# chrischoy/DeepGlobalRegistration

Measured on NVIDIA B200. Metric: scan_pairs_per_sec, higher is better.
Workload: dtype f32

## Files before the change

### deepglobalregistration_b200/csrc/knn_tc.cu

```cuda
#include <stdlib.h>

#include "common.cuh"
#include "tc_common.cuh"

namespace {

using namespace tc;

constexpr int kLoadWarps = 4;
constexpr int kLoadThreads = kLoadWarps * 32;
constexpr int kMmaWarpK = kLoadWarps;
constexpr int kEpiWarps = 8;
constexpr int kThreadsK = (kLoadWarps + 1 + kEpiWarps) * 32;
constexpr int kRowsA = 128;
constexpr int kColsB = 256;
constexpr int kATile = kRowsA * 128;
constexpr int kBTile = kColsB * 128;
constexpr int kCandCap = 16;
constexpr int kEpiThreads = kEpiWarps * 32;
constexpr size_t kCandBytes = (size_t)2 * kCandCap * kEpiThreads * 4;
constexpr int kPass1Stride = 1;

__global__ void row_norms_kernel(const float* __restrict__ f, int64_t n, int c, float* __restrict__ n2,
                                 unsigned* __restrict__ max_bits) {
  int64_t row = ((int64_t)blockIdx.x * blockDim.x + threadIdx.x) >> 3;
  int sub = threadIdx.x & 7;
  float s = 0.f;
  if (row < n)
    for (int k = sub; k < c; k += 8) {
      float v = f[row * c + k];
      s = fmaf(v, v, s);
    }
  s += __shfl_xor_sync(0xffffffffu, s, 1);
  s += __shfl_xor_sync(0xffffffffu, s, 2);
  s += __shfl_xor_sync(0xffffffffu, s, 4);
  if (row < n && sub == 0) {
    n2[row] = s;
    if (max_bits != nullptr) atomicMax(max_bits, __float_as_uint(s));
  }
}

__global__ void knn_tc_init_kernel(unsigned* __restrict__ rowmin_bits, unsigned long long* __restrict__ packed,
                                   int64_t n0, unsigned* max_bits) {
  int64_t i = (int64_t)blockIdx.x * blockDim.x + threadIdx.x;
  if (i < n0) {
    rowmin_bits[i] = 0x7f800000u;
    packed[i] = ~0ull;
  }
  if (i == 0) *max_bits = 0u;
}

__device__ __forceinline__ float knn_error_bound(float na, float nb, bool fine) {
  const float rel = fine ? 4e-6f : (0.0009765625f * 1.25f + 4e-5f);
  return rel * na * nb + 1e-6f * (na + nb) * (na + nb) + 1e-7f;
}
__global__ void knn_tc_threshold_kernel(const unsigned* __restrict__ rowmin_bits, const float* __restrict__ na2,
                                        const unsigned* __restrict__ nb2_max_bits, int64_t n0, int fine,
                                        float* __restrict__ thr) {
  int64_t i = (int64_t)blockIdx.x * blockDim.x + threadIdx.x;
  if (i >= n0) return;
  const float na = sqrtf(na2[i]), nb = sqrtf(__uint_as_float(*nb2_max_bits));
  const float e = knn_error_bound(na, nb, fine != 0);
  thr[i] = 0.5f * (__uint_as_float(rowmin_bits[i]) + 4.f * e - na2[i]);
}

struct KnnShared {
  unsigned long long full[2];
  unsigned long long acc_full[2];
  unsigned long long acc_empty[2];
  uint32_t tmem_base;
  float nb[2][kColsB];
};

__device__ __forceinline__ void round_store(float4 v, unsigned char* tile, int row, int piece) {
  float4 h;
  h.x = tf32_round(v.x); h.y = tf32_round(v.y); h.z = tf32_round(v.z); h.w = tf32_round(v.w);
  *reinterpret_cast<float4*>(tile + row * 128 + ((piece ^ (row & 7)) << 4)) = h;
}

__device__ __forceinline__ void split_store2(float4 v, unsigned char* hi_tile, unsigned char* lo_tile, int row, int piece) {
  float4 h, l;
  h.x = tf32_round(v.x); h.y = tf32_round(v.y); h.z = tf32_round(v.z); h.w = tf32_round(v.w);
  l.x = v.x - h.x; l.y = v.y - h.y; l.z = v.z - h.z; l.w = v.w - h.w;
  const int off = row * 128 + ((piece ^ (row & 7)) << 4);
  *reinterpret_cast<float4*>(hi_tile + off) = h;
  *reinterpret_cast<float4*>(lo_tile + off) = l;
}

template <int C>
__device__ __noinline__ void knn_exact_candidate(const float* __restrict__ f0, const float* __restrict__ f1,
                                                 int gi, int j, float& best_s, float& best_d2, int& best_j) {
  const float4* a = reinterpret_cast<const float4*>(f0 + (size_t)gi * C);
  const float4* b = reinterpret_cast<const float4*>(f1 + (size_t)j * C);
  float d2 = 0.f;
#pragma unroll
  for (int k = 0; k < C / 4; ++k) {
    const float4 x = __ldg(a + k), y = __ldg(b + k);
    float df = x.x - y.x; d2 = fmaf(df, df, d2);
    df = x.y - y.y; d2 = fmaf(df, df, d2);
    df = x.z - y.z; d2 = fmaf(df, df, d2);
    df = x.w - y.w; d2 = fmaf(df, df, d2);
  }
  if (d2 < best_d2) {
    const float sq = sqrtf(d2 + 1e-7f);
    if (sq < best_s) {
      best_s = sq;
      best_d2 = d2;
      best_j = j;
    }
  }
}

template <int C>
__device__ __noinline__ void knn_exact_candidate_unordered(const float* __restrict__ f0, const float* __restrict__ f1,
                                                           int gi, int j, float& best_s, float& best_d2, int& best_j) {
  const float4* a = reinterpret_cast<const float4*>(f0 + (size_t)gi * C);
  const float4* b = reinterpret_cast<const float4*>(f1 + (size_t)j * C);
  float d2 = 0.f;
#pragma unroll
  for (int k = 0; k < C / 4; ++k) {
    const float4 x = __ldg(a + k), y = __ldg(b + k);
    float df = x.x - y.x; d2 = fmaf(df, df, d2);
    df = x.y - y.y; d2 = fmaf(df, df, d2);
    df = x.z - y.z; d2 = fmaf(df, df, d2);
    df = x.w - y.w; d2 = fmaf(df, df, d2);
  }
  const float sq = sqrtf(d2 + 1e-7f);
  if (sq < best_s || (sq == best_s && j < best_j)) {
    best_s = sq;
    best_j = j;
  }
  best_d2 = fminf(best_d2, d2);
}

__device__ __forceinline__ void tc_ld32_issue(uint32_t taddr, uint32_t (&v)[32]) {
  asm volatile(
      "tcgen05.ld.sync.aligned.32x32b.x32.b32 "
      "{%0, %1, %2, %3, %4, %5, %6, %7, %8, %9, %10, %11, %12, %13, %14, %15, "
      "%16, %17, %18, %19, %20, %21, %22, %23, %24, %25, %26, %27, %28, %29, %30, %31}, [%32];"
      : "=r"(v[0]), "=r"(v[1]), "=r"(v[2]), "=r"(v[3]), "=r"(v[4]), "=r"(v[5]), "=r"(v[6]), "=r"(v[7]),
        "=r"(v[8]), "=r"(v[9]), "=r"(v[10]), "=r"(v[11]), "=r"(v[12]), "=r"(v[13]), "=r"(v[14]),
        "=r"(v[15]), "=r"(v[16]), "=r"(v[17]), "=r"(v[18]), "=r"(v[19]), "=r"(v[20]), "=r"(v[21]),
        "=r"(v[22]), "=r"(v[23]), "=r"(v[24]), "=r"(v[25]), "=r"(v[26]), "=r"(v[27]), "=r"(v[28]),
        "=r"(v[29]), "=r"(v[30]), "=r"(v[31])
      : "r"(taddr)
// ... 194 lines not shown
        atomicMin(packed + gi, ((unsigned long long)__float_as_uint(best_s) << 32) | (unsigned)best_j);
    }
  } else {
    const int lane_grp = warp & 3;
    const int half = (warp - kLoadWarps - 1) >> 2;
    const int r = lane_grp * 32 + lane;
    const int gi = row0 + r;
    const bool valid = gi < n0;
    float th = (PASS == 2 && valid) ? thr[gi] : -__int_as_float(0x7f800000);
    const float na2_i = (PASS == 2 && valid) ? na2[gi] : 0.f;
    const float e4 = (PASS == 2 && valid)
                         ? 4.f * knn_error_bound(sqrtf(na2_i), sqrtf(__uint_as_float(*nb2_max_bits)), kFine)
                         : 0.f;
    float rmin = __int_as_float(0x7f800000);
    float best_s = __int_as_float(0x7f800000), best_d2 = best_s;
    int best_j = 0x7fffffff;
    for (int it = 0; it < n_tiles; ++it) {
      const int s = it & 1;
      const uint32_t ph = (it >> 1) & 1;
      const int j0 = col_begin + it * kTS * kColsB + half * 128;
      mbar_wait(smem_u32(&sh.acc_full[s]), ph);
      tc_fence_after();
      const uint32_t taddr = tmem_base + (uint32_t)s * kColsB + half * 128 + ((uint32_t)(lane_grp * 32) << 16);
      const float* hb = sh.nb[s] + half * 128;
      uint32_t va[32], vb[32];
      tc_ld32_issue(taddr, va);
#pragma unroll
      for (int cc = 0; cc < 4; ++cc) {
        tc_ld_wait();
        uint32_t(&cur)[32] = (cc & 1) ? vb : va;
        uint32_t(&nxt)[32] = (cc & 1) ? va : vb;
        if (cc < 3) tc_ld32_issue(taddr + (cc + 1) * 32, nxt);
        const int jc = j0 + cc * 32;
        if (jc < col_end) {
          if (jc + 32 <= col_end) {
            float cmin = __int_as_float(0x7f800000);
#pragma unroll
            for (int q = 0; q < 32; ++q) cmin = fminf(cmin, hb[cc * 32 + q] - __uint_as_float(cur[q]));
            if (PASS == 1) {
              rmin = fminf(rmin, cmin);
            } else if (cmin <= th) {
#pragma unroll
              for (int q = 0; q < 32; ++q) {
                const float g = hb[cc * 32 + q] - __uint_as_float(cur[q]);
                if (g <= th) {
                  knn_exact_candidate<C>(f0, f1, gi, jc + q, best_s, best_d2, best_j);
                  th = fminf(th, 0.5f * (best_d2 + e4 - na2_i));
                }
              }
            }
          } else {
#pragma unroll
            for (int q = 0; q < 32; ++q) {
              const float g = hb[cc * 32 + q] - __uint_as_float(cur[q]);
              if (jc + q < col_end) {
                if (PASS == 1) rmin = fminf(rmin, g);
                else if (g <= th) {
                  knn_exact_candidate<C>(f0, f1, gi, jc + q, best_s, best_d2, best_j);
                  th = fminf(th, 0.5f * (best_d2 + e4 - na2_i));
                }
              }
            }
          }
        }
      }
      tc_fence_before();
      mbar_arrive(smem_u32(&sh.acc_empty[s]));
    }
    if (valid) {
      if (PASS == 1) {
        atomicMin(rowmin_bits + gi, __float_as_uint(fmaxf(fmaf(2.f, rmin, na2[gi]), 0.f)));
      } else if (best_j != 0x7fffffff) {
        atomicMin(packed + gi, ((unsigned long long)__float_as_uint(best_s) << 32) | (unsigned)best_j);
      }
    }
  }
  tc_fence_before();
  __syncthreads();
  if (warp == kMmaWarpK) {
    asm volatile("tcgen05.dealloc.cta_group::1.sync.aligned.b32 %0, %1;" ::"r"(tmem_base), "r"(512u) : "memory");
  }
}

__global__ void knn_tc_unpack_kernel(const unsigned long long* __restrict__ packed, int64_t n,
                                     int32_t* __restrict__ idx, float* __restrict__ dist) {
  int64_t i = (int64_t)blockIdx.x * blockDim.x + threadIdx.x;
  if (i >= n) return;
  unsigned long long p = packed[i];
  idx[i] = (int32_t)(p & 0xffffffffu);
  if (dist != nullptr) dist[i] = __uint_as_float((unsigned)(p >> 32));
}

template <int C>
int32_t launch_knn_tc_single(const float* f0, int64_t n0, const float* f1, int64_t n1, float* na2, float* nb2,
                             unsigned* max_bits, unsigned long long* packed, cudaStream_t st) {
  constexpr int kChunks = C / 32;
  const size_t smem = sizeof(KnnShared) + 1024 + (size_t)kChunks * kATile + 2 * (size_t)kChunks * kBTile + kCandBytes;
  DGR_ENSURE_SMEM((knn_tc_kernel<C, 3, false>), smem);
  const int row_tiles = (int)((n0 + kRowsA - 1) / kRowsA);
  const int col_tiles = (int)((n1 + kColsB - 1) / kColsB);
  int splits = (148 * 4 + row_tiles - 1) / row_tiles;
  if (splits > col_tiles) splits = col_tiles;
  if (splits < 1) splits = 1;
  const int cols_per_split = ((col_tiles + splits - 1) / splits) * kColsB;
  splits = (int)((n1 + cols_per_split - 1) / cols_per_split);
  dim3 grid(row_tiles, splits);
  knn_tc_kernel<C, 3, false><<<grid, kThreadsK, smem, st>>>(f0, (int)n0, f1, (int)n1, na2, nb2, cols_per_split,
                                                            nullptr, nullptr, packed, max_bits);
  return DGR_OK;
}

template <int C, bool kFine>
int32_t launch_knn_tc(const float* f0, int64_t n0, const float* f1, int64_t n1, float* na2, float* nb2,
                      unsigned* rowmin, float* thr, unsigned* max_bits, unsigned long long* packed,
                      cudaStream_t st) {
  constexpr int kChunks = C / 32;
  constexpr int kParts = kFine ? 2 : 1;
  const size_t smem = sizeof(KnnShared) + 1024 + (size_t)kParts * kChunks * kATile + 2 * (size_t)kParts * kChunks * kBTile;
  DGR_ENSURE_SMEM((knn_tc_kernel<C, 1, kFine>), smem);
  DGR_ENSURE_SMEM((knn_tc_kernel<C, 2, kFine>), smem);
  const int row_tiles = (int)((n0 + kRowsA - 1) / kRowsA);
  const int col_tiles = (int)((n1 + kColsB - 1) / kColsB);
  int splits = (148 * 4 + row_tiles - 1) / row_tiles;
  if (splits > col_tiles) splits = col_tiles;
  if (splits < 1) splits = 1;
  const int cols_per_split = ((col_tiles + splits - 1) / splits) * kColsB;
  splits = (int)((n1 + cols_per_split - 1) / cols_per_split);
  dim3 grid(row_tiles, splits);
  knn_tc_kernel<C, 1, kFine><<<grid, kThreadsK, smem, st>>>(f0, (int)n0, f1, (int)n1, na2, nb2, cols_per_split,
                                                            rowmin, thr, packed, max_bits);
  knn_tc_threshold_kernel<<<dgr_blocks(n0, 256), 256, 0, st>>>(rowmin, na2, max_bits, n0, kFine ? 1 : 0, thr);
  knn_tc_kernel<C, 2, kFine><<<grid, kThreadsK, smem, st>>>(f0, (int)n0, f1, (int)n1, na2, nb2, cols_per_split,
                                                            rowmin, thr, packed, max_bits);
  return DGR_OK;
}

}

extern "C" {

int64_t dgr_knn_tc_ws_elems(int64_t n0, int64_t n1) { return 3 * n0 + n1 + 8; }

int32_t dgr_knn_tc_supported(int32_t c) { return (c == 32 || c == 64) ? 1 : 0; }

int32_t dgr_knn_top1_tc(const float* f0, int64_t n0, const float* f1, int64_t n1, int32_t c,
                        uint64_t* packed_ws, float* ws, int32_t* idx, float* dist, void* stream) {
  DGR_ARG_CHECK(dgr_knn_tc_supported(c), "channel count not supported by the tensor-core kNN");
  DGR_ARG_CHECK(n1 >= 1 || n0 == 0, "F1 must not be empty");
  DGR_ARG_CHECK(n0 < (1ll << 31) && n1 < (1ll << 31), "too many rows");
  if (n0 == 0) return DGR_OK;
  cudaStream_t st = (cudaStream_t)stream;
  float* na2 = ws;
  float* thr = ws + n0;
  unsigned* rowmin = reinterpret_cast<unsigned*>(ws + 2 * n0);
  float* nb2 = ws + 3 * n0;
  unsigned* max_bits = reinterpret_cast<unsigned*>(ws + 3 * n0 + n1);
  unsigned long long* packed = reinterpret_cast<unsigned long long*>(packed_ws);
  knn_tc_init_kernel<<<dgr_blocks(n0, 256), 256, 0, st>>>(rowmin, packed, n0, max_bits);
  row_norms_kernel<<<dgr_blocks(n0 * 8, 256), 256, 0, st>>>(f0, n0, c, na2, nullptr);
  row_norms_kernel<<<dgr_blocks(n1 * 8, 256), 256, 0, st>>>(f1, n1, c, nb2, max_bits);
  static const bool coarse = getenv("DGR_KNN_FINE") == nullptr;
  static const bool single = getenv("DGR_KNN_SWEEPS") != nullptr && atoi(getenv("DGR_KNN_SWEEPS")) == 1;
  if (single) {
    int32_t rc1 = (c == 32) ? launch_knn_tc_single<32>(f0, n0, f1, n1, na2, nb2, max_bits, packed, st)
                            : launch_knn_tc_single<64>(f0, n0, f1, n1, na2, nb2, max_bits, packed, st);
    if (rc1 != DGR_OK) return rc1;
    knn_tc_unpack_kernel<<<dgr_blocks(n0, 256), 256, 0, st>>>(packed, n0, idx, dist);
    dgr_note_launches(5);
    DGR_LAUNCH_CHECK();
    return DGR_OK;
  }
  int32_t rc = (c == 32) ? (coarse ? launch_knn_tc<32, false>(f0, n0, f1, n1, na2, nb2, rowmin, thr, max_bits, packed, st)
                                   : launch_knn_tc<32, true>(f0, n0, f1, n1, na2, nb2, rowmin, thr, max_bits, packed, st))
                         : launch_knn_tc<64, false>(f0, n0, f1, n1, na2, nb2, rowmin, thr, max_bits, packed, st);
  if (rc != DGR_OK) return rc;
  knn_tc_unpack_kernel<<<dgr_blocks(n0, 256), 256, 0, st>>>(packed, n0, idx, dist);
  dgr_note_launches(7);
  DGR_LAUNCH_CHECK();
  return DGR_OK;
}

}
```

### deepglobalregistration_b200/csrc/spconv_tc.cu

```cuda
#include <cuda_fp16.h>
#include <stdlib.h>

#include "common.cuh"
#include "tc_common.cuh"

namespace {

using namespace tc;

#ifdef DGR_GATHER_CG
#define DGR_GATHER_LOAD(p) __ldcg(p)
#else
#define DGR_GATHER_LOAD(p) __ldg(p)
#endif

#define DGR_TRY_RC(expr)             \
  do {                              \
    int32_t rc__ = (expr);          \
    if (rc__ != DGR_OK) return rc__; \
  } while (0)

constexpr int kLoaderWarps = 8;
constexpr int kLoaderThreads = kLoaderWarps * 32;
constexpr int kMmaWarp = kLoaderWarps;
constexpr int kThreadsTC = (kLoaderWarps + 5) * 32;
constexpr int kTileM = 128;
constexpr int kChunk = 32;
constexpr int kATileBytes = kTileM * 128;

__device__ __forceinline__ void split_store(float4 v, unsigned char* hi_tile, unsigned char* lo_tile,
                                            uint32_t off) {
  float4 h, l;
  h.x = tf32_round(v.x); h.y = tf32_round(v.y); h.z = tf32_round(v.z); h.w = tf32_round(v.w);
  l.x = v.x - h.x; l.y = v.y - h.y; l.z = v.z - h.z; l.w = v.w - h.w;
  *reinterpret_cast<float4*>(hi_tile + off) = h;
  *reinterpret_cast<float4*>(lo_tile + off) = l;
}

__device__ __forceinline__ void split_store_f16(float4 a, float4 b, float sx, unsigned char* hi_tile,
                                                unsigned char* lo_tile, uint32_t off) {
  const float x[8] = {a.x * sx, a.y * sx, a.z * sx, a.w * sx, b.x * sx, b.y * sx, b.z * sx, b.w * sx};
  uint32_t h[4], l[4];
#pragma unroll
  for (int i = 0; i < 4; ++i) {
    const __half2 hh = __floats2half2_rn(x[2 * i], x[2 * i + 1]);
    const float2 hf = __half22float2(hh);
    const __half2 ll = __floats2half2_rn(x[2 * i] - hf.x, x[2 * i + 1] - hf.y);
    h[i] = *reinterpret_cast<const uint32_t*>(&hh);
    l[i] = *reinterpret_cast<const uint32_t*>(&ll);
  }
  *reinterpret_cast<uint4*>(hi_tile + off) = make_uint4(h[0], h[1], h[2], h[3]);
  *reinterpret_cast<uint4*>(lo_tile + off) = make_uint4(l[0], l[1], l[2], l[3]);
}
__device__ __forceinline__ float f16_scale_for(float amax) {
  const uint32_t b = __float_as_uint(amax);
  const int e = (int)((b >> 23) & 255u);
  if (e == 0 || e == 255) return 1.f;
  int se = 14 - (e - 127) + 127;
  se = se < 1 ? 1 : (se > 254 ? 254 : se);
  return __uint_as_float((uint32_t)se << 23);
}

__device__ __forceinline__ uint32_t cluster_ctarank() {
  uint32_t r;
  asm volatile("mov.u32 %0, %%cluster_ctarank;" : "=r"(r));
  return r;
}
__device__ __forceinline__ void cluster_sync_all() {
  asm volatile("barrier.cluster.arrive.release.aligned;" ::: "memory");
  asm volatile("barrier.cluster.wait.acquire.aligned;" ::: "memory");
}
__device__ __forceinline__ void bulk_g2s_multicast(uint32_t dst_smem, const void* src, uint32_t bytes,
                                                   uint32_t bar, uint16_t mask) {
  asm volatile(
      "cp.async.bulk.shared::cluster.global.mbarrier::complete_tx::bytes.multicast::cluster [%0], [%1], %2, [%3], %4;"
      ::"r"(dst_smem), "l"(src), "r"(bytes), "r"(bar), "h"(mask)
      : "memory");
}
__device__ __forceinline__ void tc_commit_multicast(uint32_t bar, uint16_t mask) {
  asm volatile(
      "tcgen05.commit.cta_group::1.mbarrier::arrive::one.shared::cluster.multicast::cluster.b64 [%0], %1;" ::"r"(bar),
      "h"(mask)
      : "memory");
}
__device__ __forceinline__ void mbar_arrive_expect_tx(uint32_t bar, uint32_t bytes) {
  asm volatile("mbarrier.arrive.expect_tx.shared::cta.b64 _, [%0], %1;" ::"r"(bar), "r"(bytes) : "memory");
}
__device__ __forceinline__ void mbar_expect_tx(uint32_t bar, uint32_t bytes) {
  asm volatile("mbarrier.expect_tx.relaxed.cta.shared::cta.b64 [%0], %1;" ::"r"(bar), "r"(bytes) : "memory");
}
__device__ __forceinline__ void bulk_g2s(uint32_t dst_smem, const void* src, uint32_t bytes, uint32_t bar) {
  asm volatile("cp.async.bulk.shared::cluster.global.mbarrier::complete_tx::bytes [%0], [%1], %2, [%3];" ::"r"(
                   dst_smem),
               "l"(src), "r"(bytes), "r"(bar)
               : "memory");
}


__device__ __forceinline__ void scatter32_lines(unsigned char* stg, int lane, float* __restrict__ out, int cout,
                                                int col, int j, const uint32_t (&v)[32]) {
#pragma unroll
  for (int q = 0; q < 8; ++q)
    *reinterpret_cast<uint4*>(stg + lane * 128 + ((q ^ (lane & 7)) << 4)) =
        make_uint4(v[4 * q], v[4 * q + 1], v[4 * q + 2], v[4 * q + 3]);
  __syncwarp();
  const int p = lane & 7, rsub = lane >> 3;
#pragma unroll
  for (int k = 0; k < 8; ++k) {
    const int R = rsub + 4 * k;
    const int jr = __shfl_sync(0xffffffffu, j, R);
    const float4 x = *reinterpret_cast<const float4*>(stg + R * 128 + ((p ^ (R & 7)) << 4));
    if (jr >= 0) red_add_v4(out + (size_t)jr * cout + col + p * 4, x.x, x.y, x.z, x.w);
  }
  __syncwarp();
}
__device__ __forceinline__ void scatter32_rows(float* __restrict__ out, int cout, int col, int j,
                                               const uint32_t (&v)[32]) {
  if (j >= 0) {
    float* dst = out + (size_t)j * cout + col;
#pragma unroll
    for (int q = 0; q < 8; ++q)
      red_add_v4(dst + 4 * q, __uint_as_float(v[4 * q]), __uint_as_float(v[4 * q + 1]),
                 __uint_as_float(v[4 * q + 2]), __uint_as_float(v[4 * q + 3]));
  }
}
constexpr int kEpiStageBytes = 4 * 4096;

struct TcShared {
  unsigned long long full[4];
  unsigned long long full_lo[4];
  unsigned long long empty[4];
  unsigned long long acc_full[2];
  unsigned long long acc_empty[2];
  uint32_t tmem_base;
};

template <int kCluster, int kPD>
__global__ void __launch_bounds__(kThreadsTC, 1)
spconv_tc_kernel(const float* __restrict__ in_feat, int cin, const float* __restrict__ wt, int cout,
                 const int32_t* __restrict__ in_idx, const int32_t* __restrict__ out_idx,
                 const int32_t* __restrict__ kofs, const int32_t* __restrict__ tile_k,
                 const int32_t* __restrict__ tile_start, int n_tiles, int n_stages, int tmem_cols,
                 int passes, int epi, float* __restrict__ out) {
  extern __shared__ __align__(16) unsigned char smem_dyn[];
  TcShared& sh = *reinterpret_cast<TcShared*>(smem_dyn);
  unsigned char* stage0 = reinterpret_cast<unsigned char*>(
      (reinterpret_cast<uintptr_t>(smem_dyn) + sizeof(TcShared) + 1023) & ~(uintptr_t)1023);
  const int b_tile_bytes = cout * 128;
  const int stage_bytes = 2 * kATileBytes + 2 * b_tile_bytes;
  const int t = threadIdx.x;
  const int warp = t >> 5, lane = t & 31;
  const int n_chunks = cin / kChunk;
  const uint32_t acc_stride = (uint32_t)tmem_cols >> 1;

  if (t == 0) {
    for (int s = 0; s < n_stages; ++s) {
      mbar_init(smem_u32(&sh.full[s]), kLoaderThreads);
      mbar_init(smem_u32(&sh.full_lo[s]), 1);
      mbar_init(smem_u32(&sh.empty[s]), kCluster);
    }
    for (int b = 0; b < 2; ++b) {
      mbar_init(smem_u32(&sh.acc_full[b]), 1);
      mbar_init(smem_u32(&sh.acc_empty[b]), 128);
    }
    asm volatile("fence.mbarrier_init.release.cluster;" ::: "memory");
  }
  if (warp == kMmaWarp) {
    asm volatile("tcgen05.alloc.cta_group::1.sync.aligned.shared::cta.b32 [%0], %1;" ::"r"(
                     smem_u32(&sh.tmem_base)),
                 "r"((uint32_t)tmem_cols)
                 : "memory");
    asm volatile("tcgen05.relinquish_alloc_permit.cta_group::1.sync.aligned;" ::: "memory");
  }
  tc_fence_before();
  __syncthreads();
  if (kCluster > 1) cluster_sync_all();
  tc_fence_after();
  const uint32_t tmem_base = sh.tmem_base;
// ... 920 lines not shown
```

### deepglobalregistration_b200/csrc/tc_common.cuh

```cuda
#pragma once
#include <cuda_runtime.h>
#include <stdint.h>

namespace tc {

__device__ __forceinline__ uint32_t smem_u32(const void* p) {
  return (uint32_t)__cvta_generic_to_shared(p);
}
__device__ __forceinline__ void mbar_init(uint32_t bar, uint32_t count) {
  asm volatile("mbarrier.init.shared::cta.b64 [%0], %1;" ::"r"(bar), "r"(count) : "memory");
}
__device__ __forceinline__ void mbar_arrive(uint32_t bar) {
  asm volatile("mbarrier.arrive.shared::cta.b64 _, [%0];" ::"r"(bar) : "memory");
}
__device__ __forceinline__ bool mbar_try_wait(uint32_t bar, uint32_t parity) {
  uint32_t ok;
  asm volatile(
      "{\n\t.reg .pred p;\n\t"
      "mbarrier.try_wait.parity.shared::cta.b64 p, [%1], %2;\n\t"
      "selp.u32 %0, 1, 0, p;\n\t}"
      : "=r"(ok)
      : "r"(bar), "r"(parity)
      : "memory");
  return ok != 0;
}
__device__ __forceinline__ void mbar_wait(uint32_t bar, uint32_t parity) {
  while (!mbar_try_wait(bar, parity)) {
  }
}
__device__ __forceinline__ void fence_proxy_async() {
  asm volatile("fence.proxy.async.shared::cta;" ::: "memory");
}
__device__ __forceinline__ void tc_fence_before() {
  asm volatile("tcgen05.fence::before_thread_sync;" ::: "memory");
}
__device__ __forceinline__ void tc_fence_after() {
  asm volatile("tcgen05.fence::after_thread_sync;" ::: "memory");
}
__device__ __forceinline__ void tc_commit(uint32_t bar) {
  asm volatile("tcgen05.commit.cta_group::1.mbarrier::arrive::one.shared::cluster.b64 [%0];" ::"r"(bar)
               : "memory");
}
__device__ __forceinline__ void tc_mma_tf32(uint32_t tmem_d, uint64_t adesc, uint64_t bdesc, uint32_t idesc,
                                            uint32_t accumulate) {
  asm volatile(
      "{\n\t.reg .pred p;\n\t"
      "setp.ne.b32 p, %4, 0;\n\t"
      "tcgen05.mma.cta_group::1.kind::tf32 [%0], %1, %2, %3, p;\n\t}"
      ::"r"(tmem_d), "l"(adesc), "l"(bdesc), "r"(idesc), "r"(accumulate)
      : "memory");
}
__device__ __forceinline__ void tc_mma_tf32_ts(uint32_t tmem_d, uint32_t tmem_a, uint64_t bdesc, uint32_t idesc,
                                               uint32_t accumulate) {
  asm volatile(
      "{\n\t.reg .pred p;\n\t"
      "setp.ne.b32 p, %4, 0;\n\t"
      "tcgen05.mma.cta_group::1.kind::tf32 [%0], [%1], %2, %3, p;\n\t}"
      ::"r"(tmem_d), "r"(tmem_a), "l"(bdesc), "r"(idesc), "r"(accumulate)
      : "memory");
}
__device__ __forceinline__ void tc_st32(uint32_t taddr, const uint32_t (&v)[32]) {
  asm volatile(
      "tcgen05.st.sync.aligned.32x32b.x32.b32 [%0], "
      "{%1, %2, %3, %4, %5, %6, %7, %8, %9, %10, %11, %12, %13, %14, %15, %16, "
      "%17, %18, %19, %20, %21, %22, %23, %24, %25, %26, %27, %28, %29, %30, %31, %32};"
      ::"r"(taddr), "r"(v[0]), "r"(v[1]), "r"(v[2]), "r"(v[3]), "r"(v[4]), "r"(v[5]), "r"(v[6]), "r"(v[7]),
        "r"(v[8]), "r"(v[9]), "r"(v[10]), "r"(v[11]), "r"(v[12]), "r"(v[13]), "r"(v[14]), "r"(v[15]),
        "r"(v[16]), "r"(v[17]), "r"(v[18]), "r"(v[19]), "r"(v[20]), "r"(v[21]), "r"(v[22]), "r"(v[23]),
        "r"(v[24]), "r"(v[25]), "r"(v[26]), "r"(v[27]), "r"(v[28]), "r"(v[29]), "r"(v[30]), "r"(v[31])
      : "memory");
}
__device__ __forceinline__ void tc_st_wait() { asm volatile("tcgen05.wait::st.sync.aligned;" ::: "memory"); }

__device__ __forceinline__ void tc_ld32(uint32_t taddr, uint32_t (&v)[32]) {
  asm volatile(
      "tcgen05.ld.sync.aligned.32x32b.x32.b32 "
      "{%0, %1, %2, %3, %4, %5, %6, %7, %8, %9, %10, %11, %12, %13, %14, %15, "
      "%16, %17, %18, %19, %20, %21, %22, %23, %24, %25, %26, %27, %28, %29, %30, %31}, [%32];"
      : "=r"(v[0]), "=r"(v[1]), "=r"(v[2]), "=r"(v[3]), "=r"(v[4]), "=r"(v[5]), "=r"(v[6]), "=r"(v[7]),
        "=r"(v[8]), "=r"(v[9]), "=r"(v[10]), "=r"(v[11]), "=r"(v[12]), "=r"(v[13]), "=r"(v[14]),
        "=r"(v[15]), "=r"(v[16]), "=r"(v[17]), "=r"(v[18]), "=r"(v[19]), "=r"(v[20]), "=r"(v[21]),
        "=r"(v[22]), "=r"(v[23]), "=r"(v[24]), "=r"(v[25]), "=r"(v[26]), "=r"(v[27]), "=r"(v[28]),
        "=r"(v[29]), "=r"(v[30]), "=r"(v[31])
      : "r"(taddr)
      : "memory");
  asm volatile("tcgen05.wait::ld.sync.aligned;" ::: "memory");
}
__device__ __forceinline__ void tc_ld16(uint32_t taddr, uint32_t (&v)[16]) {
  asm volatile(
      "tcgen05.ld.sync.aligned.32x32b.x16.b32 "
      "{%0, %1, %2, %3, %4, %5, %6, %7, %8, %9, %10, %11, %12, %13, %14, %15}, [%16];"
      : "=r"(v[0]), "=r"(v[1]), "=r"(v[2]), "=r"(v[3]), "=r"(v[4]), "=r"(v[5]), "=r"(v[6]), "=r"(v[7]),
        "=r"(v[8]), "=r"(v[9]), "=r"(v[10]), "=r"(v[11]), "=r"(v[12]), "=r"(v[13]), "=r"(v[14]),
        "=r"(v[15])
      : "r"(taddr)
      : "memory");
  asm volatile("tcgen05.wait::ld.sync.aligned;" ::: "memory");
}
__device__ __forceinline__ void red_add_v4(float* addr, float a, float b, float c, float d) {
  asm volatile("red.global.add.v4.f32 [%0], {%1, %2, %3, %4};" ::"l"(addr), "f"(a), "f"(b), "f"(c), "f"(d)
               : "memory");
}
__device__ __forceinline__ float tf32_round(float x) {
  uint32_t r;
  asm("cvt.rna.tf32.f32 %0, %1;" : "=r"(r) : "f"(x));
  return __uint_as_float(r);
}

__device__ __forceinline__ uint64_t umma_desc(uint32_t smem_addr) {
  uint64_t d = 0;
  d |= (uint64_t)((smem_addr & 0x3FFFFu) >> 4);
  d |= (uint64_t)1 << 16;
  d |= (uint64_t)(1024 >> 4) << 32;
  d |= (uint64_t)1 << 46;
  d |= (uint64_t)2 << 61;
  return d;
}


}
```

Measured before the change: 117.4.

## Add FP16 tensor-core kNN path with per-row scaling and persistent pipelined kernel

Adds a new default kNN path that packs features into scaled FP16 swizzled images and runs a persistent tcgen05 f16 MMA kernel. The kernel uses a multi-stage bulk-copy pipeline for B tiles, double-buffered A tiles and TMEM accumulators. It keeps the two-pass threshold scheme with an FP16-aware error bound and exact rescoring of candidates. The aim is to halve the operand bytes and raise MMA throughput compared with TF32. The cost is extra pack kernels, more workspace, and a looser error bound that may send more candidates to exact rescoring.

After: 122.8, median of 6. 1.05x the previous value.

```diff
diff --git a/deepglobalregistration_b200/csrc/knn_tc.cu b/deepglobalregistration_b200/csrc/knn_tc.cu
--- a/deepglobalregistration_b200/csrc/knn_tc.cu
+++ b/deepglobalregistration_b200/csrc/knn_tc.cu
@@ -1,3 +1,4 @@
+#include <cuda_fp16.h>
 #include <stdlib.h>
 
 #include "common.cuh"
@@ -25,18 +26,25 @@
                                  unsigned* __restrict__ max_bits) {
   int64_t row = ((int64_t)blockIdx.x * blockDim.x + threadIdx.x) >> 3;
   int sub = threadIdx.x & 7;
-  float s = 0.f;
+  float s = 0.f, amax = 0.f;
   if (row < n)
     for (int k = sub; k < c; k += 8) {
       float v = f[row * c + k];
       s = fmaf(v, v, s);
+      amax = fmaxf(amax, fabsf(v));
     }
   s += __shfl_xor_sync(0xffffffffu, s, 1);
   s += __shfl_xor_sync(0xffffffffu, s, 2);
   s += __shfl_xor_sync(0xffffffffu, s, 4);
+  amax = fmaxf(amax, __shfl_xor_sync(0xffffffffu, amax, 1));
+  amax = fmaxf(amax, __shfl_xor_sync(0xffffffffu, amax, 2));
+  amax = fmaxf(amax, __shfl_xor_sync(0xffffffffu, amax, 4));
   if (row < n && sub == 0) {
     n2[row] = s;
-    if (max_bits != nullptr) atomicMax(max_bits, __float_as_uint(s));
+    if (max_bits != nullptr) {
+      atomicMax(max_bits, __float_as_uint(s));
+      atomicMax(max_bits + 1, __float_as_uint(amax));
+    }
   }
 }
 
@@ -47,20 +55,26 @@
     rowmin_bits[i] = 0x7f800000u;
     packed[i] = ~0ull;
   }
-  if (i == 0) *max_bits = 0u;
+  if (i == 0) max_bits[0] = max_bits[1] = 0u;
 }
 
 __device__ __forceinline__ float knn_error_bound(float na, float nb, bool fine) {
   const float rel = fine ? 4e-6f : (0.0009765625f * 1.25f + 4e-5f);
   return rel * na * nb + 1e-6f * (na + nb) * (na + nb) + 1e-7f;
 }
+__device__ __forceinline__ float knn_error_bound_f16(float na, float nb, float inv_sa, float inv_sb, int c) {
+  const float rc = sqrtf((float)c);
+  return knn_error_bound(na, nb, false) + 3.1e-8f * rc * (na * inv_sb + nb * inv_sa) +
+         (float)c * 1e-15f * inv_sa * inv_sb;
+}
 __global__ void knn_tc_threshold_kernel(const unsigned* __restrict__ rowmin_bits, const float* __restrict__ na2,
                                         const unsigned* __restrict__ nb2_max_bits, int64_t n0, int fine,
-                                        float* __restrict__ thr) {
+                                        const float* __restrict__ inv_s0, int c, float* __restrict__ thr) {
   int64_t i = (int64_t)blockIdx.x * blockDim.x + threadIdx.x;
   if (i >= n0) return;
   const float na = sqrtf(na2[i]), nb = sqrtf(__uint_as_float(*nb2_max_bits));
-  const float e = knn_error_bound(na, nb, fine != 0);
+  const float e = inv_s0 != nullptr ? knn_error_bound_f16(na, nb, inv_s0[i], __uint_as_float(nb2_max_bits[2]), c)
+                                    : knn_error_bound(na, nb, fine != 0);
   thr[i] = 0.5f * (__uint_as_float(rowmin_bits[i]) + 4.f * e - na2[i]);
 }
 
@@ -421,6 +435,238 @@
   }
 }
 
+constexpr int kRowsH = 256;
+constexpr int kColsH = 128;
+constexpr int kStagesH = 6;
+constexpr int kAImgH = kRowsH * 128;
+constexpr int kBImgH = kColsH * 128;
+constexpr int kThreadsH = (2 + kEpiWarps) * 32;
+
+struct KnnSharedH {
+  float nb[kStagesH][kColsH];
+  unsigned long long full[kStagesH];
+  unsigned long long empty[kStagesH];
+  unsigned long long a_full[2], a_empty[2];
+  unsigned long long acc_full[2], acc_empty[2];
+  uint32_t tmem_base;
+};
+
+template <int C>
+__global__ void knn_pack_f16_kernel(const float* __restrict__ f, int64_t n, int64_t n_pad,
+                                    const unsigned* __restrict__ amax_bits, float* __restrict__ inv_scale,
+                                    const float* __restrict__ n2, float* __restrict__ nbh, uint4* __restrict__ img) {
+  const int64_t row = ((int64_t)blockIdx.x * blockDim.x + threadIdx.x) >> 3;
+  const int p = threadIdx.x & 7;
+  if (row >= n_pad) return;
+  float x[8] = {0.f, 0.f, 0.f, 0.f, 0.f, 0.f, 0.f, 0.f};
+  if (row < n && p * 8 < C) {
+    const float4 u = __ldg(reinterpret_cast<const float4*>(f + row * C + p * 8));
+    const float4 v = __ldg(reinterpret_cast<const float4*>(f + row * C + p * 8 + 4));
+    x[0] = u.x; x[1] = u.y; x[2] = u.z; x[3] = u.w; x[4] = v.x; x[5] = v.y; x[6] = v.z; x[7] = v.w;
+  }
+  float am;
+  if (amax_bits == nullptr) {
+    am = 0.f;
+#pragma unroll
+    for (int k = 0; k < 8; ++k) am = fmaxf(am, fabsf(x[k]));
+    am = fmaxf(am, __shfl_xor_sync(0xffffffffu, am, 1));
+    am = fmaxf(am, __shfl_xor_sync(0xffffffffu, am, 2));
+    am = fmaxf(am, __shfl_xor_sync(0xffffffffu, am, 4));
+  } else {
+    am = __uint_as_float(*amax_bits);
+  }
+  const float sc = f16_scale_for(am);
+  uint32_t h[4];
+#pragma unroll
+  for (int k = 0; k < 4; ++k) {
+    const __half2 hh = __floats2half2_rn(x[2 * k] * sc, x[2 * k + 1] * sc);
+    h[k] = *reinterpret_cast<const uint32_t*>(&hh);
+  }
+  img[row * 8 + (p ^ (int)(row & 7))] = make_uint4(h[0], h[1], h[2], h[3]);
+  if (p == 0) {
+    if (amax_bits == nullptr) {
+      inv_scale[row] = 1.f / sc;
+    } else {
+      if (row == 0) inv_scale[0] = 1.f / sc;
+      nbh[row] = row < n ? 0.5f * n2[row] : __int_as_float(0x7f800000);
+    }
+  }
+}
+
+template <int C, int PASS>
+__global__ void __launch_bounds__(kThreadsH, 1)
+knn_f16_kernel(const unsigned char* __restrict__ a_img, const unsigned char* __restrict__ b_img,
+               const float* __restrict__ nbh, int n0, int n1, int n_ct, int64_t n_units,
+               const float* __restrict__ f0, const float* __restrict__ f1, const float* __restrict__ na2,
+               const float* __restrict__ inv_s0, const unsigned* __restrict__ max_bits,
+               unsigned* __restrict__ rowmin_bits, const float* __restrict__ thr,
+               unsigned long long* __restrict__ packed) {
+  extern __shared__ __align__(16) unsigned char smem_dyn[];
+  KnnSharedH& sh = *reinterpret_cast<KnnSharedH*>(smem_dyn);
+  unsigned char* a_buf = reinterpret_cast<unsigned char*>(
+      (reinterpret_cast<uintptr_t>(smem_dyn) + sizeof(KnnSharedH) + 1023) & ~(uintptr_t)1023);
+  unsigned char* b_buf = a_buf + 2 * kAImgH;
+  const int t = threadIdx.x, warp = t >> 5, lane = t & 31;
+  const int64_t u_begin = (int64_t)blockIdx.x * n_units / gridDim.x;
+  const int64_t u_end = (int64_t)(blockIdx.x + 1) * n_units / gridDim.x;
+
+  if (t == 0) {
+    for (int s = 0; s < kStagesH; ++s) {
+      mbar_init(smem_u32(&sh.full[s]), 1);
+      mbar_init(smem_u32(&sh.empty[s]), kEpiWarps * 32);
+    }
+    for (int b = 0; b < 2; ++b) {
+      mbar_init(smem_u32(&sh.a_full[b]), 1);
+      mbar_init(smem_u32(&sh.a_empty[b]), 1);
+      mbar_init(smem_u32(&sh.acc_full[b]), 1);
+      mbar_init(smem_u32(&sh.acc_empty[b]), kEpiWarps * 32);
+    }
+    asm volatile("fence.mbarrier_init.release.cluster;" ::: "memory");
+  }
+  if (warp == 1) {
+    asm volatile("tcgen05.alloc.cta_group::1.sync.aligned.shared::cta.b32 [%0], %1;" ::"r"(
+                     smem_u32(&sh.tmem_base)),
+                 "r"(512u)
+                 : "memory");
+    asm volatile("tcgen05.relinquish_alloc_permit.cta_group::1.sync.aligned;" ::: "memory");
+  }
+  tc_fence_before();
+  __syncthreads();
+  tc_fence_after();
+  const uint32_t tmem_base = sh.tmem_base;
+
+  if (warp == 0) {
+    if (lane == 0) {
+      int it = 0, seg = 0;
+      for (int64_t u = u_begin; u < u_end; ++u, ++it) {
+        const int rt = (int)(u / n_ct), ct = (int)(u % n_ct);
+        if (u == u_begin || ct == 0) {
+          const int a = seg & 1;
+          mbar_wait(smem_u32(&sh.a_empty[a]), ((seg >> 1) & 1) ^ 1);
+          mbar_arrive_expect_tx(smem_u32(&sh.a_full[a]), kAImgH);
+          bulk_g2s(smem_u32(a_buf + a * kAImgH), a_img + (size_t)rt * kAImgH, kAImgH, smem_u32(&sh.a_full[a]));
+          ++seg;
+        }
+        const int s = it % kStagesH;
+        mbar_wait(smem_u32(&sh.empty[s]), ((it / kStagesH) & 1) ^ 1);
+        mbar_arrive_expect_tx(smem_u32(&sh.full[s]), kBImgH + kColsH * 4);
+        bulk_g2s(smem_u32(b_buf + s * kBImgH), b_img + (size_t)ct * kBImgH, kBImgH, smem_u32(&sh.full[s]));
+        bulk_g2s(smem_u32(sh.nb[s]), nbh + (size_t)ct * kColsH, kColsH * 4, smem_u32(&sh.full[s]));
+      }
+    }
+  } else if (warp == 1) {
+    const uint32_t idesc = (1u << 4) | ((uint32_t)(kColsH >> 3) << 17) | ((uint32_t)(128 >> 4) << 24);
+    int it = 0, seg = 0, a = 0;
+    for (int64_t u = u_begin; u < u_end; ++u, ++it) {
+      const int ct = (int)(u % n_ct);
+      if (u == u_begin || ct == 0) {
+        a = seg & 1;
+        mbar_wait(smem_u32(&sh.a_full[a]), (seg >> 1) & 1);
+        ++seg;
+      }
+      const int b = it & 1, s = it % kStagesH;
+      mbar_wait(smem_u32(&sh.acc_empty[b]), ((it >> 1) & 1) ^ 1);
+      mbar_wait(smem_u32(&sh.full[s]), (it / kStagesH) & 1);
+      tc_fence_after();
+      if (lane == 0) {
+        const uint32_t a0 = smem_u32(a_buf + a * kAImgH), b0 = smem_u32(b_buf + s * kBImgH);
+        const uint32_t td = tmem_base + (uint32_t)b * 256;
+#pragma unroll
+        for (int ks = 0; ks < C / 16; ++ks) {
+          const uint64_t bd = umma_desc(b0 + ks * 32);
+          tc_mma_f16(td, umma_desc(a0 + ks * 32), bd, idesc, ks != 0);
+          tc_mma_f16(td + 128, umma_desc(a0 + kAImgH / 2 + ks * 32), bd, idesc, ks != 0);
+        }
+        tc_commit(smem_u32(&sh.acc_full[b]));
+        if (u + 1 == u_end || ct == n_ct - 1) tc_commit(smem_u32(&sh.a_empty[a]));
+      }
+      __syncwarp();
+    }
+  } else {
+    const int lane_grp = warp & 3;
+    const int mh = (warp - 2) >> 2;
+    const int r = mh * 128 + lane_grp * 32 + lane;
+    const float pinf = __int_as_float(0x7f800000);
+    const float inv_s1 = __uint_as_float(max_bits[2]);
+    const float nb_max = sqrtf(__uint_as_float(max_bits[0]));
+    int gi = 0;
+    bool valid = false;
+    float inv = 0.f, th = -pinf, na2_i = 0.f, e4 = 0.f, rmin = pinf, best_s = pinf, best_d2 = pinf;
+    int best_j = 0x7fffffff;
+    int it = 0;
+    for (int64_t u = u_begin; u < u_end; ++u, ++it) {
+      const int rt = (int)(u / n_ct), ct = (int)(u % n_ct);
+      if (u == u_begin || ct == 0) {
+        gi = rt * kRowsH + r;
+        valid = gi < n0;
+        inv = valid ? inv_s0[gi] * inv_s1 : 0.f;
+        rmin = pinf; best_s = pinf; best_d2 = pinf; best_j = 0x7fffffff;
+        if (PASS == 2) {
+          th = valid ? thr[gi] : -pinf;
+          na2_i = valid ? na2[gi] : 0.f;
+          e4 = valid ? 4.f * knn_error_bound_f16(sqrtf(na2_i), nb_max, inv_s0[gi], inv_s1, C) : 0.f;
+        }
+      }
+      const int b = it & 1, s = it % kStagesH;
+      mbar_wait(smem_u32(&sh.acc_full[b]), (it >> 1) & 1);
+      mbar_wait(smem_u32(&sh.full[s]), (it / kStagesH) & 1);
+      tc_fence_after();
+      const uint32_t taddr = tmem_base + (uint32_t)b * 256 + mh * 128 + ((uint32_t)(lane_grp * 32) << 16);
+      const float4* hb = reinterpret_cast<const float4*>(sh.nb[s]);
+      const int j0 = ct * kColsH;
+      uint32_t va[32], vb[32];
+      tc_ld32_issue(taddr, va);
+#pragma unroll
+      for (int cc = 0; cc < 4; ++cc) {
+        tc_ld_wait();
+        uint32_t(&cur)[32] = (cc & 1) ? vb : va;
+        uint32_t(&nxt)[32] = (cc & 1) ? va : vb;
+        if (cc < 3) tc_ld32_issue(taddr + (cc + 1) * 32, nxt);
+        const int jc = j0 + cc * 32;
+        if (jc < n1) {
+          float g[32];
+#pragma unroll
+          for (int q4 = 0; q4 < 8; ++q4) {
+            const float4 h4 = hb[cc * 8 + q4];
+            g[4 * q4 + 0] = fmaf(-__uint_as_float(cur[4 * q4 + 0]), inv, h4.x);
+            g[4 * q4 + 1] = fmaf(-__uint_as_float(cur[4 * q4 + 1]), inv, h4.y);
+            g[4 * q4 + 2] = fmaf(-__uint_as_float(cur[4 * q4 + 2]), inv, h4.z);
+            g[4 * q4 + 3] = fmaf(-__uint_as_float(cur[4 * q4 + 3]), inv, h4.w);
+          }
+          float cmin = pinf;
+#pragma unroll
+          for (int q = 0; q < 32; ++q) cmin = fminf(cmin, g[q]);
+          if (PASS == 1) {
+            rmin = fminf(rmin, cmin);
+          } else if (cmin <= th) {
+            const int nq = min(32, n1 - jc);
+#pragma unroll
+            for (int q = 0; q < 32; ++q) {
+              if (q < nq && g[q] <= th) {
+                knn_exact_candidate<C>(f0, f1, gi, jc + q, best_s, best_d2, best_j);
+                th = fminf(th, 0.5f * (best_d2 + e4 - na2_i));
+              }
+            }
+          }
+        }
+      }
+      tc_fence_before();
+      mbar_arrive(smem_u32(&sh.acc_empty[b]));
+      mbar_arrive(smem_u32(&sh.empty[s]));
+      if (valid && (u + 1 == u_end || ct == n_ct - 1)) {
+        if (PASS == 1) atomicMin(rowmin_bits + gi, __float_as_uint(fmaxf(fmaf(2.f, rmin, na2[gi]), 0.f)));
+        else if (best_j != 0x7fffffff)
+          atomicMin(packed + gi, ((unsigned long long)__float_as_uint(best_s) << 32) | (unsigned)best_j);
+      }
+    }
+  }
+  tc_fence_before();
+  __syncthreads();
+  if (warp == 1) {
+    asm volatile("tcgen05.dealloc.cta_group::1.sync.aligned.b32 %0, %1;" ::"r"(tmem_base), "r"(512u) : "memory");
+  }
+}
+
 __global__ void knn_tc_unpack_kernel(const unsigned long long* __restrict__ packed, int64_t n,
                                      int32_t* __restrict__ idx, float* __restrict__ dist) {
   int64_t i = (int64_t)blockIdx.x * blockDim.x + threadIdx.x;
@@ -428,6 +674,56 @@
   unsigned long long p = packed[i];
   idx[i] = (int32_t)(p & 0xffffffffu);
   if (dist != nullptr) dist[i] = __uint_as_float((unsigned)(p >> 32));
+}
+
+struct KnnWs {
+  int64_t n0p, n1p, base, inv_s0, nbh, a_img, b_img, total;
+  KnnWs(int64_t n0, int64_t n1) {
+    n0p = (n0 + kRowsH - 1) / kRowsH * kRowsH;
+    n1p = (n1 + kColsH - 1) / kColsH * kColsH;
+    base = (3 * n0 + n1 + 8 + 63) / 64 * 64;
+    inv_s0 = base;
+    nbh = inv_s0 + n0p;
+    a_img = nbh + n1p;
+    b_img = a_img + n0p * 32;
+    total = b_img + n1p * 32;
+  }
+};
+
+int sm_count() {
+  int dev = 0, n = 0;
+  if (cudaGetDevice(&dev) != cudaSuccess || cudaDeviceGetAttribute(&n, cudaDevAttrMultiProcessorCount, dev) != cudaSuccess)
+    return 148;
+  return n;
+}
+
+template <int C>
+int32_t launch_knn_f16(const float* f0, int64_t n0, const float* f1, int64_t n1, float* ws, unsigned* rowmin,
+                       float* thr, unsigned* max_bits, unsigned long long* packed, cudaStream_t st) {
+  const KnnWs w(n0, n1);
+  float* na2 = ws;
+  float* nb2 = ws + 3 * n0;
+  float* inv_s0 = ws + w.inv_s0;
+  float* nbh = ws + w.nbh;
+  unsigned char* a_img = reinterpret_cast<unsigned char*>(ws + w.a_img);
+  unsigned char* b_img = reinterpret_cast<unsigned char*>(ws + w.b_img);
+  knn_pack_f16_kernel<C><<<dgr_blocks(w.n0p * 8, 256), 256, 0, st>>>(f0, n0, w.n0p, nullptr, inv_s0, nullptr, nullptr,
+                                                                       reinterpret_cast<uint4*>(a_img));
+  knn_pack_f16_kernel<C><<<dgr_blocks(w.n1p * 8, 256), 256, 0, st>>>(
+      f1, n1, w.n1p, max_bits + 1, reinterpret_cast<float*>(max_bits + 2), nb2, nbh, reinterpret_cast<uint4*>(b_img));
+  const size_t smem = sizeof(KnnSharedH) + 1024 + 2 * (size_t)kAImgH + (size_t)kStagesH * kBImgH;
+  DGR_ENSURE_SMEM((knn_f16_kernel<C, 1>), smem);
+  DGR_ENSURE_SMEM((knn_f16_kernel<C, 2>), smem);
+  const int n_ct = (int)(w.n1p / kColsH);
+  const int64_t n_units = (w.n0p / kRowsH) * n_ct;
+  static const int n_sm = sm_count();
+  const int grid = (int)(n_units < n_sm ? n_units : n_sm);
+  knn_f16_kernel<C, 1><<<grid, kThreadsH, smem, st>>>(a_img, b_img, nbh, (int)n0, (int)n1, n_ct, n_units, f0, f1, na2,
+                                                      inv_s0, max_bits, rowmin, thr, packed);
+  knn_tc_threshold_kernel<<<dgr_blocks(n0, 256), 256, 0, st>>>(rowmin, na2, max_bits, n0, 0, inv_s0, C, thr);
+  knn_f16_kernel<C, 2><<<grid, kThreadsH, smem, st>>>(a_img, b_img, nbh, (int)n0, (int)n1, n_ct, n_units, f0, f1, na2,
+                                                      inv_s0, max_bits, rowmin, thr, packed);
+  return DGR_OK;
 }
 
 template <int C>
@@ -468,7 +764,8 @@
   dim3 grid(row_tiles, splits);
   knn_tc_kernel<C, 1, kFine><<<grid, kThreadsK, smem, st>>>(f0, (int)n0, f1, (int)n1, na2, nb2, cols_per_split,
                                                             rowmin, thr, packed, max_bits);
-  knn_tc_threshold_kernel<<<dgr_blocks(n0, 256), 256, 0, st>>>(rowmin, na2, max_bits, n0, kFine ? 1 : 0, thr);
+  knn_tc_threshold_kernel<<<dgr_blocks(n0, 256), 256, 0, st>>>(rowmin, na2, max_bits, n0, kFine ? 1 : 0, nullptr,
+                                                               C, thr);
   knn_tc_kernel<C, 2, kFine><<<grid, kThreadsK, smem, st>>>(f0, (int)n0, f1, (int)n1, na2, nb2, cols_per_split,
                                                             rowmin, thr, packed, max_bits);
   return DGR_OK;
@@ -478,7 +775,7 @@
 
 extern "C" {
 
-int64_t dgr_knn_tc_ws_elems(int64_t n0, int64_t n1) { return 3 * n0 + n1 + 8; }
+int64_t dgr_knn_tc_ws_elems(int64_t n0, int64_t n1) { return KnnWs(n0, n1).total; }
 
 int32_t dgr_knn_tc_supported(int32_t c) { return (c == 32 || c == 64) ? 1 : 0; }
 
@@ -498,6 +795,17 @@
   knn_tc_init_kernel<<<dgr_blocks(n0, 256), 256, 0, st>>>(rowmin, packed, n0, max_bits);
   row_norms_kernel<<<dgr_blocks(n0 * 8, 256), 256, 0, st>>>(f0, n0, c, na2, nullptr);
   row_norms_kernel<<<dgr_blocks(n1 * 8, 256), 256, 0, st>>>(f1, n1, c, nb2, max_bits);
+  const char* tf32_env = getenv("DGR_KNN_TF32");
+  const bool tf32 = tf32_env != nullptr && atoi(tf32_env) == 1;
+  if (!tf32) {
+    int32_t rc = (c == 32) ? launch_knn_f16<32>(f0, n0, f1, n1, ws, rowmin, thr, max_bits, packed, st)
+                           : launch_knn_f16<64>(f0, n0, f1, n1, ws, rowmin, thr, max_bits, packed, st);
+    if (rc != DGR_OK) return rc;
+    knn_tc_unpack_kernel<<<dgr_blocks(n0, 256), 256, 0, st>>>(packed, n0, idx, dist);
+    dgr_note_launches(9);
+    DGR_LAUNCH_CHECK();
+    return DGR_OK;
+  }
   static const bool coarse = getenv("DGR_KNN_FINE") == nullptr;
   static const bool single = getenv("DGR_KNN_SWEEPS") != nullptr && atoi(getenv("DGR_KNN_SWEEPS")) == 1;
   if (single) {
diff --git a/deepglobalregistration_b200/csrc/spconv_tc.cu b/deepglobalregistration_b200/csrc/spconv_tc.cu
--- a/deepglobalregistration_b200/csrc/spconv_tc.cu
+++ b/deepglobalregistration_b200/csrc/spconv_tc.cu
@@ -52,14 +52,6 @@
   *reinterpret_cast<uint4*>(hi_tile + off) = make_uint4(h[0], h[1], h[2], h[3]);
   *reinterpret_cast<uint4*>(lo_tile + off) = make_uint4(l[0], l[1], l[2], l[3]);
 }
-__device__ __forceinline__ float f16_scale_for(float amax) {
-  const uint32_t b = __float_as_uint(amax);
-  const int e = (int)((b >> 23) & 255u);
-  if (e == 0 || e == 255) return 1.f;
-  int se = 14 - (e - 127) + 127;
-  se = se < 1 ? 1 : (se > 254 ? 254 : se);
-  return __uint_as_float((uint32_t)se << 23);
-}
 
 __device__ __forceinline__ uint32_t cluster_ctarank() {
   uint32_t r;
@@ -82,18 +74,6 @@
       "tcgen05.commit.cta_group::1.mbarrier::arrive::one.shared::cluster.multicast::cluster.b64 [%0], %1;" ::"r"(bar),
       "h"(mask)
       : "memory");
-}
-__device__ __forceinline__ void mbar_arrive_expect_tx(uint32_t bar, uint32_t bytes) {
-  asm volatile("mbarrier.arrive.expect_tx.shared::cta.b64 _, [%0], %1;" ::"r"(bar), "r"(bytes) : "memory");
-}
-__device__ __forceinline__ void mbar_expect_tx(uint32_t bar, uint32_t bytes) {
-  asm volatile("mbarrier.expect_tx.relaxed.cta.shared::cta.b64 [%0], %1;" ::"r"(bar), "r"(bytes) : "memory");
-}
-__device__ __forceinline__ void bulk_g2s(uint32_t dst_smem, const void* src, uint32_t bytes, uint32_t bar) {
-  asm volatile("cp.async.bulk.shared::cluster.global.mbarrier::complete_tx::bytes [%0], [%1], %2, [%3];" ::"r"(
-                   dst_smem),
-               "l"(src), "r"(bytes), "r"(bar)
-               : "memory");
 }
 
 
diff --git a/deepglobalregistration_b200/csrc/tc_common.cuh b/deepglobalregistration_b200/csrc/tc_common.cuh
--- a/deepglobalregistration_b200/csrc/tc_common.cuh
+++ b/deepglobalregistration_b200/csrc/tc_common.cuh
@@ -28,6 +28,18 @@
   while (!mbar_try_wait(bar, parity)) {
   }
 }
+__device__ __forceinline__ void mbar_arrive_expect_tx(uint32_t bar, uint32_t bytes) {
+  asm volatile("mbarrier.arrive.expect_tx.shared::cta.b64 _, [%0], %1;" ::"r"(bar), "r"(bytes) : "memory");
+}
+__device__ __forceinline__ void mbar_expect_tx(uint32_t bar, uint32_t bytes) {
+  asm volatile("mbarrier.expect_tx.relaxed.cta.shared::cta.b64 [%0], %1;" ::"r"(bar), "r"(bytes) : "memory");
+}
+__device__ __forceinline__ void bulk_g2s(uint32_t dst_smem, const void* src, uint32_t bytes, uint32_t bar) {
+  asm volatile("cp.async.bulk.shared::cluster.global.mbarrier::complete_tx::bytes [%0], [%1], %2, [%3];" ::"r"(
+                   dst_smem),
+               "l"(src), "r"(bytes), "r"(bar)
+               : "memory");
+}
 __device__ __forceinline__ void fence_proxy_async() {
   asm volatile("fence.proxy.async.shared::cta;" ::: "memory");
 }
@@ -47,6 +59,15 @@
       "{\n\t.reg .pred p;\n\t"
       "setp.ne.b32 p, %4, 0;\n\t"
       "tcgen05.mma.cta_group::1.kind::tf32 [%0], %1, %2, %3, p;\n\t}"
+      ::"r"(tmem_d), "l"(adesc), "l"(bdesc), "r"(idesc), "r"(accumulate)
+      : "memory");
+}
+__device__ __forceinline__ void tc_mma_f16(uint32_t tmem_d, uint64_t adesc, uint64_t bdesc, uint32_t idesc,
+                                           uint32_t accumulate) {
+  asm volatile(
+      "{\n\t.reg .pred p;\n\t"
+      "setp.ne.b32 p, %4, 0;\n\t"
+      "tcgen05.mma.cta_group::1.kind::f16 [%0], %1, %2, %3, p;\n\t}"
       ::"r"(tmem_d), "l"(adesc), "l"(bdesc), "r"(idesc), "r"(accumulate)
       : "memory");
 }
@@ -107,6 +128,15 @@
   return __uint_as_float(r);
 }
 
+__device__ __forceinline__ float f16_scale_for(float amax) {
+  const uint32_t b = __float_as_uint(amax);
+  const int e = (int)((b >> 23) & 255u);
+  if (e == 0 || e == 255) return 1.f;
+  int se = 14 - (e - 127) + 127;
+  se = se < 1 ? 1 : (se > 254 ? 254 : se);
+  return __uint_as_float((uint32_t)se << 23);
+}
+
 __device__ __forceinline__ uint64_t umma_desc(uint32_t smem_addr) {
   uint64_t d = 0;
   d |= (uint64_t)((smem_addr & 0x3FFFFu) >> 4);
```
